# LiuTaowen-Tony/xKV

Measured on NVIDIA B200. Metric: KV GB/s compressed (prefill, xKV-4, Llama-3.1-8B 64K), higher is better.
Workload: dtype bf16

## Files before the change

include/xkv_b200.h:

```cpp
#ifndef XKV_B200_H_
#define XKV_B200_H_

#include <stddef.h>
#include <stdint.h>

#ifdef __cplusplus
extern "C" {
#endif

#if defined(__GNUC__)
#define XKV_API __attribute__((visibility("default")))
#else
#define XKV_API
#endif

#define XKV_MAX_GROUP_LAYERS 16
#define XKV_MAX_GEMM_PROBLEMS 16
#define XKV_MAX_BATCH 16
#define XKV_MAX_LAYER_MAPS 64

XKV_API const char* xkv_last_error(void);
XKV_API int xkv_version(void);
XKV_API int64_t xkv_launch_count(void);

// ... 5 lines not shown
                     void* stream);

typedef struct xkv_gemm_problem {
  int32_t M, N, K;
  int32_t num_terms;
  int32_t a_mn_major;
  int32_t b_mn_major;
  const void* A[3];
  const void* B[3];
  int64_t lda, ldb;
  uint8_t term_a[6], term_b[6];
  void* D;
  int64_t ldd;
  int32_t out_bf16;
  int32_t out_transposed;
  int32_t sym_upper;
  int32_t split_k;
  int64_t split_stride;
  int32_t accum_phases;
  const int32_t* run_if;
  int32_t a_layers, b_layers, layer_cols;
  const void* A_layer[XKV_MAX_GROUP_LAYERS];
  const void* B_layer[XKV_MAX_GROUP_LAYERS];
} xkv_gemm_problem;
XKV_API int xkv_gemm_grouped(const xkv_gemm_problem* problems_host, int num_problems, void* stream);
XKV_API size_t xkv_gemm_problem_size(void);
XKV_API void xkv_gemm_set_gram_pair(int on);

XKV_API int xkv_reduce_slabs(const float* slabs, int num_slabs, int64_t slab_stride, int rows, int cols, int64_t ld,
                     int symmetrize, float* out, int64_t ld_out, void* stream);
XKV_API int xkv_reduce_slabs_batched(const float* const* slabs_host, float* const* out_host, int batch, int num_slabs,
                                     int64_t slab_stride, int rows, int cols, int64_t ld, int symmetrize,
                                     int64_t ld_out, void* stream);
XKV_API int xkv_split_bf16(const float* x, int rows, int cols, int64_t ld, void* hi, void* mid, void* lo,
                   int64_t ld_out, void* stream);
XKV_API int xkv_split_bf16_batched(const float* const* x_host, void* const* hi_host, void* const* mid_host,
                                   void* const* lo_host, int batch, int rows, int cols, int64_t ld, int64_t ld_out,
                                   void* stream);
XKV_API int xkv_symmetrize_split_bf16(const float* const* slabs_host, int batch, int num_slabs, int64_t slab_stride,
                                      int n, int64_t ld, void* const* hi_host, void* const* mid_host,
                                      void* const* lo_host, int64_t ld_out, void* stream);
XKV_API size_t xkv_gram_packed_elems(int n);
XKV_API int xkv_gram_pack_upper(const float* full, int n, int64_t ld, float* packed, void* stream);
XKV_API int xkv_gram_unpack_upper(const float* packed, int n, float* full, int64_t ld, void* stream);
XKV_API int xkv_fill_gaussian_bf16(void* out, int rows, int cols, int64_t ld, uint64_t seed, void* stream);
XKV_API int xkv_normalize_rows(float* const* Y_host, void* const* hi_host, void* const* mid_host,
                               void* const* lo_host, int batch, int rows, int cols, int64_t ld, int64_t ld_out,
                               void* stream);
XKV_API int xkv_shift_normalize_rows(float* const* Y_host, const float* const* Q_host, float* shift_dev,
                                     float* const* rdiag_host, int rdiag_first, void* const* hi_host,
// ... 120 lines not shown
```

xkv_b200/_lib.py:

```python
from __future__ import annotations

import ctypes as C
import os
from typing import Optional

_LIB_PATH = os.environ.get("XKV_B200_LIB") or os.path.join(os.path.dirname(os.path.abspath(__file__)), "libxkv_b200.so")
_lib: Optional[C.CDLL] = None

MAX_GROUP_LAYERS = 16
MAX_GEMM_PROBLEMS = 16
MAX_BATCH = 16


class XkvError(RuntimeError):
    """Raised when a C-ABI call returns a non-zero status (mirrors the reference's Python exceptions)."""


class GemmProblem(C.Structure):

    _fields_ = [
        ("M", C.c_int32),
        ("N", C.c_int32),
        ("K", C.c_int32),
        ("num_terms", C.c_int32),
        ("a_mn_major", C.c_int32),
        ("b_mn_major", C.c_int32),
        ("A", C.c_void_p * 3),
        ("B", C.c_void_p * 3),
        ("lda", C.c_int64),
        ("ldb", C.c_int64),
        ("term_a", C.c_uint8 * 6),
        ("term_b", C.c_uint8 * 6),
        ("D", C.c_void_p),
        ("ldd", C.c_int64),
        ("out_bf16", C.c_int32),
        ("out_transposed", C.c_int32),
        ("sym_upper", C.c_int32),
        ("split_k", C.c_int32),
        ("split_stride", C.c_int64),
        ("accum_phases", C.c_int32),
        ("run_if", C.c_void_p),
        ("a_layers", C.c_int32),
        ("b_layers", C.c_int32),
        ("layer_cols", C.c_int32),
        ("A_layer", C.c_void_p * MAX_GROUP_LAYERS),
        ("B_layer", C.c_void_p * MAX_GROUP_LAYERS),
    ]


class AppendProblem(C.Structure):

    _fields_ = [("x_new", C.c_void_p), ("V", C.c_void_p), ("a_out", C.c_void_p), ("ldx", C.c_int64), ("ldv", C.c_int64),
                ("lda", C.c_int64), ("n", C.c_int32), ("r", C.c_int32)]


class FactorizeOptions(C.Structure):

    _fields_ = [
        ("power_iters", C.c_int32),
        ("oversample", C.c_int32),
        ("first_passes", C.c_int32),
        ("passes", C.c_int32),
        ("final_passes", C.c_int32),
        ("window", C.c_int32),
        ("jacobi_sweeps", C.c_int32),
        ("rayleigh_ritz", C.c_int32),
        ("want_sigma", C.c_int32),
        ("gram_split_k", C.c_int32),
        ("gram_chunk_tokens", C.c_int32),
# ... 45 lines not shown
    "xkv_convert_bf16": (_i, [_vp, _i, _i, _i64, _vp, _i64, _vp, _i64, _vp]),
    "xkv_sqrt_clamp": (_i, [_vp, _vp, _i, _vp]),
    "xkv_factorize_default_options": (None, [C.POINTER(FactorizeOptions)]),
    "xkv_factorize_workspace_bytes": (_sz, [_i, _i, _i, _i, C.POINTER(FactorizeOptions)]),
    "xkv_factorize_sigma_count": (_i, [_i, C.POINTER(FactorizeOptions)]),
    "xkv_decode_workspace_bytes": (_sz, [_i, _i, _i, _i]),
    "xkv_decode_attention": (_i, [_vp, _i, _i, _i, _vp, _i64, _i, _vp, _i64, _vp, _i64, _i, _vp, _i64, _i, _vp, _vp, _i64,
                                  _vp, _vp, _i, _i64, _i64, _f, _vp, _vp, _sz, _vp]),
    "xkv_decode_attention_lse": (_i, [_vp, _i, _i, _i, _vp, _i64, _i, _vp, _i64, _vp, _i64, _i, _vp, _i64, _i, _vp, _vp,
                                      _i64, _vp, _vp, _i, _i64, _i64, _f, _vp, _vp, _sz, _vp, _vp]),
    "xkv_decode_absorbed_workspace_bytes": (_sz, [_i, _i, _i]),
    "xkv_decode_absorbed": (_i, [_vp, _i, _vp, _i64, _i, _i, _vp, _vp, _vp, _i64, _i, _f, _vp, _vp, _vp, _sz, _vp]),
    "xkv_decode_force_tiled": (None, [_i]),
    "xkv_decode_set_variant": (None, [_i]),
    "xkv_decode_set_stages": (None, [_i]),
    "xkv_rope_bf16": (_i, [_vp, _i64, _i, _i, _i, _vp, _vp, _i64, _vp]),
    "xkv_append_workspace_bytes": (_sz, [_i, _i, _i]),
    "xkv_append_project": (_i, [_vp, _i64, _i, _vp, _i64, _i, _i, _vp, _i64, _vp, _sz, _vp]),
    "xkv_append_project_batch": (_i, [C.POINTER(AppendProblem), _i, _i, _vp, _sz, _vp]),
    "xkv_slerp_workspace_bytes": (_sz, [_i64]),
    "xkv_slerp_merge": (_i, [_vp, _vp, _i64, _i, _i64, _f, _f, _vp, _vp, _i64, _vp, _sz, _vp]),
    "xkv_gemm_problem_size": (C.c_size_t, []),
    "xkv_gemm_set_gram_pair": (None, [_i]),
    "xkv_factorize_groups": (_i, [_pp, _i, _i, _i, _i, _i64, _i, C.POINTER(FactorizeOptions), _pp, _pp, _pp, _pp, _vp, _sz,
                                  _pp, _vp]),
    "xkv_factorize_workspace_bytes_mixed": (_sz, [_i, _i, _i, _vp, C.POINTER(FactorizeOptions)]),
    "xkv_factorize_groups_mixed": (_i, [_pp, _i, _i, _i, _i, _i64, _vp, C.POINTER(FactorizeOptions), _pp, _pp, _pp, _pp, _vp,
                                        _sz, _pp, _vp]),
    "xkv_factorize_batch_mixed": (_i, [_pp, _i, _i, _i, _i64, _vp, C.POINTER(FactorizeOptions), _pp, _pp, _pp, _pp, _vp, _sz,
                                       _pp, _vp]),
    "xkv_factorize_batch": (_i, [_pp, _i, _i, _i, _i64, _i, C.POINTER(FactorizeOptions), _pp, _pp, _pp, _pp, _pp, _i,
                                 _vp, _sz, _pp, _vp]),
}


def lib_path() -> str:
    return _LIB_PATH


def load() -> C.CDLL:
    global _lib
    if _lib is not None:
        return _lib
    if not os.path.exists(_LIB_PATH):
        raise XkvError(
            f"{_LIB_PATH} not found: build it with `python -c 'import __graft_entry__ as g; g.build()'` "
# ... 16 lines not shown
```

xkv_b200/csrc/xkv_factorize.cu:

```cuda
#include <cuda_bf16.h>

#include <vector>

#include "xkv_host.h"

namespace xkv {

static inline size_t align_up(size_t x, size_t a) { return (x + a - 1) / a * a; }
static inline int round_up_int(int x, int k) { return (x + k - 1) / k * k; }

struct Bump {
  char* base;
  size_t off, cap;
  bool overflow;
  void* take(size_t bytes) {
    off = align_up(off, 1024);
    void* p = base ? base + off : nullptr;
    off += bytes;
    if (base && off > cap) overflow = true;
    return p;
  }
  float* f32(size_t n) { return static_cast<float*>(take(n * 4)); }
  void* bf16(size_t n) { return take(n * 2); }
};
// ... 411 lines not shown
                                               o.pivot_floor, stream));
          }
          if (o.heavy_redo && pp > 0 && shift < o.shifts[0]) {
            BatchRowsScope rows(l_rows);
            XKV_TRY(xkv_pass_flags(P.linv, B, lmax, lmax, 2.f * shift, P.redo_flags, stream));
            xkv_set_launch_predicate(P.redo_flags);
            int rc2 = xkv_reduce_slabs_batched(P.s_slabs, P.s_mat, B, P.sk, static_cast<long long>(lmax) * lmax, lmax, lmax, lmax,
                                               1, lmax, stream);
            if (!rc2)
              rc2 = xkv_cholesky_inverse_limbs(P.s_mat, P.linv, h0, h1, nt > 3 ? h2 : nullptr, B, lmax, lmax, lmax, o.shifts[0],
                                               o.pivot_floor, stream);
            xkv_set_launch_predicate(cond ? P.pass_flags : nullptr);
            if (rc2) return rc2;
          }
        }
        if (track) {
          BatchRowsScope rows(l_rows);
          XKV_TRY(xkv_rdiag_update(P.rdiag, P.linv, B, lmax, lmax, stream));
        }
        for (int b = 0; b < B; ++b) {
          xkv_gemm_problem p = swap_roles(problem(P.linv_l[b][0], P.linv_l[b][1], P.linv_l[b][2], lmax, 0, P.lh[b], P.lm[b],
                                                  P.ll[b], nn, 1, cond ? cur[b] : nxt[b], nn, l[b], n, l[b],
                                                  (o.solve_terms == 3 && !final_call) ? 3 : nt));
          p.run_if = cond ? P.pass_flags + b : nullptr;
          ps.push_back(p);
        }
        XKV_TRY(run_gemms(ps, stream));
        return 0;
      }();
      if (cond) xkv_set_launch_predicate(nullptr);
      if (rc) return rc;
      if (!cond) swap_bufs();
    }
    return 0;
  };
  auto apply_gram = [&](int nterms) -> int {
    for (int b = 0; b < B; ++b)
      ps.push_back(swap_roles(problem(P.lh[b], P.lm[b], P.ll[b], nn, 0, P.g_limb[b][0], P.g_limb[b][1], P.g_limb[b][2], nn, 0,
                                      nxt[b], nn, l[b], n, n, nterms)));
    XKV_TRY(run_gemms(ps, stream));
    swap_bufs();
    return 0;
  };

  for (int b = 0; b < B; ++b) XKV_TRY(xkv_fill_gaussian_bf16(P.lh[b], l[b], n, nn, o.seed + 7919ull * b, stream));
  XKV_TRY(apply_gram(1));
// ... 175 lines not shown
```

xkv_b200/csrc/xkv_gemm.cu:

```cuda
#include <cstdlib>

#include "xkv_common.cuh"
#include "xkv_host.h"

namespace xkv {

constexpr int BM = 128;
constexpr int BN = 256;
constexpr int BK = 64;
constexpr int STAGES = 4;
constexpr int A_TILE_BYTES = BM * BK * 2;
constexpr int B_TILE_BYTES = BN * BK * 2;
constexpr int STAGE_BYTES = A_TILE_BYTES + B_TILE_BYTES;
constexpr int CHUNK_BYTES = 64 * BK * 2;
constexpr int GEMM_THREADS = 192;
constexpr int TMEM_COLS = 256;
constexpr size_t GEMM_SMEM_BYTES = STAGES * STAGE_BYTES + 1024  + 256 ;

struct alignas(64) GemmProb {
  CUtensorMap a_map[3];
  CUtensorMap b_map[3];
  void* D;
  long long ldd;
  long long split_stride;
  int M, N, K;
  int nterms;
  int tiles_m, tiles_n, ntiles;
  int split_k, kblocks_per_split, nkb;
  int cta_begin;
  int bn;
  int na, nb;
  unsigned char la[3], lb[3];
  unsigned char sa[3], sb[3];
  int pstages;
  int out_bf16, out_transposed, sym_upper;
  unsigned char ta[6], tb[6];
  const int* run_if;
  int phases;
  int a_layers, a_layer_begin, b_layers, b_layer_begin, layer_cols;
};
struct GemmParams {
  int nprob;
  int pair_stages;
  GemmProb p[XKV_MAX_GEMM_PROBLEMS];
  CUtensorMap layer_maps[XKV_MAX_LAYER_MAPS];
};

__device__ __forceinline__ const CUtensorMap* layer_map(const GemmParams& P, int begin, int layers, int layer_cols, int col,
                                                        int& col_in_layer) {
  int li = col / layer_cols;
  li = li < layers ? li : layers - 1;
  col_in_layer = col - li * layer_cols;
  return &P.layer_maps[begin + li];
}

template <int A_MN, int B_MN>
__global__ void __launch_bounds__(GEMM_THREADS, 1) gemm_kernel(const __grid_constant__ GemmParams P) {
  extern __shared__ uint8_t smem_raw[];
  uint8_t* smem = reinterpret_cast<uint8_t*>((reinterpret_cast<uintptr_t>(smem_raw) + 1023) & ~uintptr_t(1023));
  uint64_t* full_bar = reinterpret_cast<uint64_t*>(smem + STAGES * STAGE_BYTES);
  uint64_t* empty_bar = full_bar + STAGES;
  uint64_t* tmem_full_bar = empty_bar + STAGES;
  uint64_t* tmem_empty_bar = tmem_full_bar + 2;
  uint32_t* tmem_slot = reinterpret_cast<uint32_t*>(tmem_empty_bar + 2);

  const int warp = threadIdx.x >> 5;
  const int lane = threadIdx.x & 31;

  int pi = 0;
  while (pi + 1 < P.nprob && static_cast<int>(blockIdx.x) >= P.p[pi + 1].cta_begin) ++pi;
  const GemmProb& pr = P.p[pi];
  if (pr.run_if != nullptr && *pr.run_if == 0) return;
  const int local = static_cast<int>(blockIdx.x) - pr.cta_begin;
  const int split = local / pr.ntiles;
  int t = local - split * pr.ntiles;
  int tm, tn;
  if (pr.sym_upper) {
    tm = 0;
    tn = 0;
    for (int i = 0; i < pr.tiles_m; ++i) {
      const int first = (i * BM) / BN;
      const int cnt = pr.tiles_n - first;
      if (t < cnt) {
        tm = i;
        tn = first + t;
        break;
      }
      t -= cnt;
    }
  } else {
    tm = t / pr.tiles_n;
    tn = t - tm * pr.tiles_n;
  }
  const int m0 = tm * BM;
  const int n0 = tn * BN;
  const int kb0 = split * pr.kblocks_per_split;
  const int kb1 = min(kb0 + pr.kblocks_per_split, pr.nkb);
  const int nk = max(kb1 - kb0, 0);
  const int niter = nk * pr.nterms;
  const int nph = max(1, min(pr.phases, nk));
  const uint32_t tmem_cols = nph > 1 ? 2 * TMEM_COLS : TMEM_COLS;

  if (warp == 0 && lane == 0) {
    for (int i = 0; i < STAGES; ++i) {
      mbar_init(&full_bar[i], 1);
      mbar_init(&empty_bar[i], 1);
    }
    mbar_init(&tmem_full_bar[0], 1);
    mbar_init(&tmem_full_bar[1], 1);
    mbar_init(&tmem_empty_bar[0], 4);
    mbar_init(&tmem_empty_bar[1], 4);
    mbar_fence_init();
    for (int i = 0; i < 3; ++i) {
      tma_prefetch_desc(&pr.a_map[i]);
      tma_prefetch_desc(&pr.b_map[i]);
    }
  }
  if (warp == 1) tmem_alloc(tmem_slot, tmem_cols);
  tc_fence_before();
  __syncthreads();
  tc_fence_after();
  const uint32_t tmem_base = *tmem_slot;

  if (warp == 0) {
    const CUtensorMap* a_chunk_map[BM / 64];
    int a_chunk_col[BM / 64];
    const CUtensorMap* b_chunk_map[BN / 64];
    int b_chunk_col[BN / 64];
#pragma unroll
    for (int c = 0; c < BM / 64; ++c) {
      a_chunk_col[c] = m0 + 64 * c;
      a_chunk_map[c] = (A_MN && pr.a_layers) ? layer_map(P, pr.a_layer_begin, pr.a_layers, pr.layer_cols, m0 + 64 * c, a_chunk_col[c]) : nullptr;
    }
#pragma unroll
    for (int c = 0; c < BN / 64; ++c) {
      b_chunk_col[c] = n0 + 64 * c;
      b_chunk_map[c] = (B_MN && pr.b_layers) ? layer_map(P, pr.b_layer_begin, pr.b_layers, pr.layer_cols, n0 + 64 * c, b_chunk_col[c]) : nullptr;
    }
    int ka_layer = 0, ka_col = 0, kb_layer = 0, kb_col = 0;
    if (!A_MN && pr.a_layers) {
      ka_layer = (kb0 * BK) / pr.layer_cols;
      ka_col = kb0 * BK - ka_layer * pr.layer_cols;
    }
    if (!B_MN && pr.b_layers) {
      kb_layer = (kb0 * BK) / pr.layer_cols;
      kb_col = kb0 * BK - kb_layer * pr.layer_cols;
    }
    if (elect_one()) {
      int s = 0, term = 0, kb = kb0;
      uint32_t ph = 0;
      for (int it = 0; it < niter; ++it) {
        const CUtensorMap* amap = &pr.a_map[pr.ta[term]];
        const CUtensorMap* bmap = &pr.b_map[pr.tb[term]];
        uint8_t* sA = smem + s * STAGE_BYTES;
        uint8_t* sB = sA + A_TILE_BYTES;
        mbar_wait(&empty_bar[s], ph ^ 1u);
        mbar_expect_tx(&full_bar[s], STAGE_BYTES);
        if (A_MN == 0) {
          if (pr.a_layers)
            tma_load_2d(sA, &P.layer_maps[pr.a_layer_begin + min(ka_layer, pr.a_layers - 1)], &full_bar[s],
                        ka_layer < pr.a_layers ? ka_col : pr.layer_cols, m0);
          else
            tma_load_2d(sA, amap, &full_bar[s], kb * BK, m0);
        } else {
#pragma unroll
          for (int c = 0; c < BM / 64; ++c)
            tma_load_2d(sA + c * CHUNK_BYTES, a_chunk_map[c] ? a_chunk_map[c] : amap, &full_bar[s], a_chunk_col[c], kb * BK);
        }
        if (B_MN == 0) {
          if (pr.b_layers)
            tma_load_2d(sB, &P.layer_maps[pr.b_layer_begin + min(kb_layer, pr.b_layers - 1)], &full_bar[s],
                        kb_layer < pr.b_layers ? kb_col : pr.layer_cols, n0);
          else
            tma_load_2d(sB, bmap, &full_bar[s], kb * BK, n0);
        } else {
#pragma unroll
          for (int c = 0; c < BN / 64; ++c)
            tma_load_2d(sB + c * CHUNK_BYTES, b_chunk_map[c] ? b_chunk_map[c] : bmap, &full_bar[s], b_chunk_col[c], kb * BK);
        }
        if (!A_MN && pr.a_layers && (ka_col += BK) >= pr.layer_cols) {
          ka_col -= pr.layer_cols;
          ++ka_layer;
        }
        if (!B_MN && pr.b_layers && (kb_col += BK) >= pr.layer_cols) {
          kb_col -= pr.layer_cols;
          ++kb_layer;
        }
        if (++term == pr.nterms) {
          term = 0;
          ++kb;
        }
        if (++s == STAGES) {
          s = 0;
          ph ^= 1u;
        }
      }
    }
    __syncwarp();
  } else if (warp == 1) {
    constexpr uint32_t idesc = umma_idesc_bf16(BM, BN, A_MN, B_MN);
    constexpr uint64_t kStageStep = STAGE_BYTES >> 4;
    constexpr uint64_t kAStep = (A_MN ? 2048 : 32) >> 4, kBStep = (B_MN ? 2048 : 32) >> 4;
    if (elect_one()) {
      const uint32_t a_base0 = smem_u32(smem);
      const uint64_t a_desc0 = A_MN ? umma_desc_sw128(a_base0, CHUNK_BYTES, 1024) : umma_desc_sw128(a_base0, 16, 1024);
      const uint64_t b_desc0 = B_MN ? umma_desc_sw128(a_base0 + A_TILE_BYTES, CHUNK_BYTES, 1024)
                                    : umma_desc_sw128(a_base0 + A_TILE_BYTES, 16, 1024);
      uint64_t a_desc = a_desc0, b_desc = b_desc0;
      int s = 0;
      uint32_t ph = 0;
      int it = 0;
      for (int phs = 0; phs < nph; ++phs) {
        const uint32_t acc = tmem_base + static_cast<uint32_t>(phs & 1) * TMEM_COLS;
        if (phs >= 2) {
          mbar_wait(&tmem_empty_bar[phs & 1], static_cast<uint32_t>(((phs >> 1) - 1) & 1));
          tc_fence_after();
        }
        const int it_end = (nph == 1) ? niter : static_cast<int>((static_cast<long long>(nk) * (phs + 1)) / nph) * pr.nterms;
        const int it_begin = it;
        for (; it < it_end; ++it) {
          mbar_wait(&full_bar[s], ph);
          tc_fence_after();
          umma_bf16_ss(acc, a_desc, b_desc, idesc, it > it_begin ? 1u : 0u);
          umma_bf16_ss(acc, a_desc + kAStep, b_desc + kBStep, idesc, 1u);
          umma_bf16_ss(acc, a_desc + 2 * kAStep, b_desc + 2 * kBStep, idesc, 1u);
          umma_bf16_ss(acc, a_desc + 3 * kAStep, b_desc + 3 * kBStep, idesc, 1u);
          umma_commit(&empty_bar[s]);
          a_desc += kStageStep;
          b_desc += kStageStep;
          if (++s == STAGES) {
            s = 0;
            ph ^= 1u;
            a_desc = a_desc0;
            b_desc = b_desc0;
          }
        }
        umma_commit(&tmem_full_bar[phs & 1]);
      }
    }
    __syncwarp();
  } else {
    const int q = warp & 3;
    const int row = m0 + q * 32 + lane;
    const bool row_ok = row < pr.M;
    float* outf = reinterpret_cast<float*>(pr.D) + static_cast<long long>(split) * pr.split_stride;
    __nv_bfloat16* outh = reinterpret_cast<__nv_bfloat16*>(pr.D) + static_cast<long long>(split) * pr.split_stride;
    const bool vec_ok = (pr.ldd % 8 == 0) && ((reinterpret_cast<uintptr_t>(pr.D) & 15) == 0) &&
                        ((pr.split_stride % 8) == 0);
#pragma unroll 1
    for (int phs = 0; phs < nph; ++phs) {
    float4 pre[8];
    auto prefetch = [&](int c) -> bool {
      const int col0 = n0 + c * 32;
      if (!(phs > 0 && row_ok && vec_ok && c < BN / 32 && col0 + 32 <= pr.N)) return false;
      const float4* src = reinterpret_cast<const float4*>(outf + static_cast<long long>(row) * pr.ldd + col0);
#pragma unroll
      for (int j = 0; j < 8; ++j) pre[j] = src[j];
      return true;
    };
    bool have_pre = prefetch(0);
    mbar_wait(&tmem_full_bar[phs & 1], static_cast<uint32_t>((phs >> 1) & 1));
    tc_fence_after();
    const uint32_t acc = tmem_base + static_cast<uint32_t>(phs & 1) * TMEM_COLS;
#pragma unroll 1
    for (int c = 0; c < BN / 32; ++c) {
      const int col0 = n0 + c * 32;
      if (col0 >= pr.N) break;
      uint32_t v[32];
      __syncwarp();
      if (niter > 0) {
        tmem_ld_32x32(acc + (static_cast<uint32_t>(q * 32) << 16) + static_cast<uint32_t>(c * 32), v);
        float4 cur[8];
        const bool have_cur = have_pre;
#pragma unroll
        for (int j = 0; j < 8; ++j) cur[j] = pre[j];
        have_pre = prefetch(c + 1);
        tmem_ld_wait();
        if (have_cur) {
#pragma unroll
          for (int j = 0; j < 8; ++j) {
            v[4 * j] = __float_as_uint(__uint_as_float(v[4 * j]) + cur[j].x);
            v[4 * j + 1] = __float_as_uint(__uint_as_float(v[4 * j + 1]) + cur[j].y);
            v[4 * j + 2] = __float_as_uint(__uint_as_float(v[4 * j + 2]) + cur[j].z);
            v[4 * j + 3] = __float_as_uint(__uint_as_float(v[4 * j + 3]) + cur[j].w);
          }
        } else if (phs > 0 && row_ok) {
          const float* src = outf + static_cast<long long>(row) * pr.ldd + col0;
#pragma unroll
// ... 100 lines not shown
  const int local = (static_cast<int>(blockIdx.x) - pr.cta_begin) >> 1;
  const int split = local / pr.ntiles;
  int t = local - split * pr.ntiles;
  int tm = 0, tn = 0;
  if (pr.sym_upper) {
    for (int i = 0; i < pr.tiles_m; ++i) {
      const int cnt = pr.tiles_n - i;
      if (t < cnt) {
        tm = i;
        tn = i + t;
        break;
      }
      t -= cnt;
    }
  } else {
    tm = t / pr.tiles_n;
    tn = t - tm * pr.tiles_n;
  }
  const int m0 = tm * PG_BM + crank * BM;
  const int n0 = tn * bn;
  const int nb0 = n0 + crank * (bn >> 1);
  const int n_end = min(pr.N, n0 + bn);
  const int kb0 = split * pr.kblocks_per_split;
  const int kb1 = min(kb0 + pr.kblocks_per_split, pr.nkb);
  const int nk = max(kb1 - kb0, 0);
  const int niter = nk * pr.nterms;
  const int nph = max(1, min(pr.phases, nk));
  const uint32_t tmem_cols = nph > 1 ? 2 * TMEM_COLS : TMEM_COLS;
  const uint32_t b_bytes = B_MN ? static_cast<uint32_t>(PG_B_BYTES) : static_cast<uint32_t>(bn >> 1) * (BK * 2);

  if (warp == 0 && lane == 0) {
    for (int i = 0; i < nstages; ++i) {
      mbar_init(&full_bar[i], 1);
      mbar_init(&empty_bar[i], 1);
    }
    mbar_init(&tmem_full_bar[0], 1);
    mbar_init(&tmem_full_bar[1], 1);
    mbar_init(&tmem_empty_bar[0], 8);
    mbar_init(&tmem_empty_bar[1], 8);
    mbar_fence_init();
    tma_prefetch_desc(&pr.a_map[pr.ta[0]]);
    tma_prefetch_desc(&pr.b_map[pr.tb[0]]);
  }
  if (warp == 1) tmem_alloc_pair(tmem_slot, tmem_cols);
  tc_fence_before();
  __syncthreads();
  cluster_sync_all();
// ... 225 lines not shown
              if (row_ok && col0 + j < n_end)
                outh[static_cast<long long>(col0 + j) * pr.ldd + row] = __float2bfloat16_rn(__uint_as_float(v[j]));
          }
        }
      }
      if (phs + 2 < nph) {
        tc_fence_before();
        __syncwarp();
        if (lane == 0) mbar_arrive_cluster(tempty0 + static_cast<uint32_t>((phs & 1) * 8));
      }
    }
  }

  tc_fence_before();
  __syncthreads();
  cluster_sync_all();
  if (warp == 1) {
    tc_fence_after();
    tmem_dealloc_pair(tmem_base, tmem_cols);
  }
}

static int g_gram_pair = 1;

static int pair_bn(const xkv_gemm_problem& p) {
  if (!g_gram_pair) return 0;
  const int rem = p.M % PG_BM;
  if (!(p.M >= 2048 || rem == 0 || rem > BM)) return 0;
  if (p.sym_upper) return (p.a_mn_major && p.b_mn_major && p.M == p.N) ? BN : 0;
  if (p.b_mn_major) return BN;
  const int ntn = (p.N + BN - 1) / BN;
  const int w = (p.N + ntn - 1) / ntn;
  return (w + 15) & ~15;
}

static int build_problem(const xkv_gemm_problem& in, GemmProb& out, int& cta_cursor, GemmParams& params, int& map_cursor,
                         int pair_n = 0) {
  const bool pair = pair_n > 0;
  const int bn = pair ? pair_n : BN;
  XKV_REQUIRE(in.M > 0 && in.N > 0 && in.K > 0, "gemm: empty problem M=%d N=%d K=%d", in.M, in.N, in.K);
  XKV_REQUIRE(in.num_terms >= 1 && in.num_terms <= 6, "gemm: num_terms=%d out of range", in.num_terms);
  XKV_REQUIRE(in.lda % 8 == 0 && in.ldb % 8 == 0, "gemm: lda/ldb must be multiples of 8 elements");
  XKV_REQUIRE(in.split_k >= 1, "gemm: split_k must be >= 1");
  XKV_REQUIRE(in.D != nullptr, "gemm: null output");
  std::memset(&out, 0, sizeof(out));
  bool used_a[3] = {false, false, false}, used_b[3] = {false, false, false};
  for (int t = 0; t < in.num_terms; ++t) {
    XKV_REQUIRE(in.term_a[t] < 3 && in.term_b[t] < 3, "gemm: limb index out of range");
    used_a[in.term_a[t]] = true;
    used_b[in.term_b[t]] = true;
    out.ta[t] = in.term_a[t];
    out.tb[t] = in.term_b[t];
  }
  XKV_REQUIRE(in.a_layers >= 0 && in.a_layers <= XKV_MAX_GROUP_LAYERS && in.b_layers >= 0 && in.b_layers <= XKV_MAX_GROUP_LAYERS,
              "gemm: at most %d layers per operand", XKV_MAX_GROUP_LAYERS);
  if (in.a_layers > 0 || in.b_layers > 0) {
    XKV_REQUIRE(in.num_terms == 1, "gemm: layered operands take one term");
    XKV_REQUIRE(in.layer_cols > 0 && in.layer_cols % 64 == 0, "gemm: layer_cols=%d must be a positive multiple of 64", in.layer_cols);
  }
  for (int side = 0; side < 2; ++side) {
    const int layers = side == 0 ? in.a_layers : in.b_layers;
    if (layers == 0) continue;
    const void* const* ptrs = side == 0 ? in.A_layer : in.B_layer;
    const bool mn = side == 0 ? in.a_mn_major != 0 : in.b_mn_major != 0;
    const long long ld = side == 0 ? in.lda : in.ldb;
    const int other = side == 0 ? in.M : in.N;
    if (side == 1 && in.a_layers == in.b_layers && in.a_mn_major && in.b_mn_major && in.lda == in.ldb &&
        std::memcmp(in.A_layer, in.B_layer, sizeof(void*) * layers) == 0) {
      out.b_layer_begin = out.a_layer_begin;
      continue;
    }
    (side == 0 ? out.a_layer_begin : out.b_layer_begin) = map_cursor;
    for (int i = 0; i < layers; ++i) {
      XKV_REQUIRE(ptrs[i] != nullptr && (reinterpret_cast<uintptr_t>(ptrs[i]) & 15) == 0, "gemm: layer %d null or unaligned", i);
      XKV_REQUIRE(map_cursor < XKV_MAX_LAYER_MAPS, "gemm: more than %d layer matrices in one launch", XKV_MAX_LAYER_MAPS);
      int rc;
      if (!mn)
        rc = encode_tmap_2d_bf16(&params.layer_maps[map_cursor++], ptrs[i], in.layer_cols, other, ld, BK,
                                 side == 0 ? BM : (pair ? bn / 2 : BN));
      else
        rc = encode_tmap_2d_bf16(&params.layer_maps[map_cursor++], ptrs[i], in.layer_cols, in.K, ld, 64, BK);
      if (rc) return rc;
    }
  }
  out.a_layers = in.a_layers;
  out.b_layers = in.b_layers;
  out.layer_cols = in.layer_cols;
  XKV_REQUIRE(in.a_layers == 0 || (in.a_mn_major ? in.M : in.K) <= in.a_layers * in.layer_cols, "gemm: layered A narrower than the problem");
  XKV_REQUIRE(in.b_layers == 0 || (in.b_mn_major ? in.N : in.K) <= in.b_layers * in.layer_cols, "gemm: layered B narrower than the problem");
  for (int i = 0; i < 3; ++i) {
    const void* a = in.a_layers > 0 ? in.A_layer[0] : (used_a[i] ? in.A[i] : in.A[in.term_a[0]]);
    const void* b = in.b_layers > 0 ? in.B_layer[0] : (used_b[i] ? in.B[i] : in.B[in.term_b[0]]);
    XKV_REQUIRE(a != nullptr && b != nullptr, "gemm: null operand limb %d", i);
    XKV_REQUIRE((reinterpret_cast<uintptr_t>(a) & 15) == 0 && (reinterpret_cast<uintptr_t>(b) & 15) == 0,
                "gemm: operands must be 16-byte aligned");
    int rc = 0;
    if (in.a_layers > 0)
      out.a_map[i] = params.layer_maps[out.a_layer_begin];
    else if (!in.a_mn_major)
      rc = encode_tmap_2d_bf16(&out.a_map[i], a, in.K, in.M, in.lda, BK, BM);
    else
      rc = encode_tmap_2d_bf16(&out.a_map[i], a, in.M, in.K, in.lda, 64, BK);
    if (rc) return rc;
    if (in.b_layers > 0)
      out.b_map[i] = params.layer_maps[out.b_layer_begin];
    else if (!in.b_mn_major)
      rc = encode_tmap_2d_bf16(&out.b_map[i], b, in.K, in.N, in.ldb, BK, pair ? bn / 2 : BN);
    else
      rc = encode_tmap_2d_bf16(&out.b_map[i], b, in.N, in.K, in.ldb, 64, BK);
    if (rc) return rc;
  }
  out.D = in.D;
  out.ldd = in.ldd;
  out.split_stride = in.split_stride;
  out.M = in.M;
  out.N = in.N;
  out.K = in.K;
  out.nterms = in.num_terms;
  const int bm = pair ? PG_BM : BM;
  out.bn = bn;
  out.tiles_m = (in.M + bm - 1) / bm;
  out.tiles_n = (in.N + bn - 1) / bn;
  out.sym_upper = in.sym_upper ? 1 : 0;
  if (out.sym_upper) {
    int cnt = 0;
    for (int i = 0; i < out.tiles_m; ++i) cnt += out.tiles_n - (i * bm) / bn;
    out.ntiles = cnt;
  } else {
    out.ntiles = out.tiles_m * out.tiles_n;
  }
  for (int i = 0; i < 3; ++i) {
    if (used_a[i]) {
      out.sa[i] = static_cast<unsigned char>(out.na);
      out.la[out.na++] = static_cast<unsigned char>(i);
    }
    if (used_b[i]) {
      out.sb[i] = static_cast<unsigned char>(out.nb);
      out.lb[out.nb++] = static_cast<unsigned char>(i);
    }
  }
  out.nkb = (in.K + BK - 1) / BK;
  out.split_k = in.split_k;
  out.kblocks_per_split = (out.nkb + in.split_k - 1) / in.split_k;
  out.out_bf16 = in.out_bf16 ? 1 : 0;
  out.out_transposed = in.out_transposed ? 1 : 0;
  out.run_if = in.run_if;
  out.phases = in.accum_phases > 1 ? in.accum_phases : 1;
  XKV_REQUIRE(out.phases == 1 || (!in.out_bf16 && !in.out_transposed),
              "gemm: accum_phases > 1 needs a plain fp32 output");
  out.cta_begin = cta_cursor;
  cta_cursor += out.ntiles * out.split_k * (pair ? 2 : 1);
  return 0;
}

bool& gemm_low_priority() {
  static thread_local bool low = false;
  return low;
}

template <int A_MN, int B_MN>
static int launch_pair_variant(GemmParams& params, int grid, cudaStream_t stream) {
  auto kern = gemm_pair_kernel<A_MN, B_MN>;
  static PerDevice<bool> configured;
  if (!configured()) {
    XKV_CHECK_CUDA(cudaFuncSetAttribute(kern, cudaFuncAttributeMaxDynamicSharedMemorySize,
                                        static_cast<int>(pg_smem_bytes(PG_MAX_STAGES))));
    configured() = true;
  }
  params.pair_stages = (g_gram_pair >= 3 && g_gram_pair <= PG_MAX_STAGES) ? g_gram_pair : PG_STAGES;
  for (int i = 0; i < params.nprob; ++i) {
    const int stage = (params.p[i].na + params.p[i].nb) * PG_A_BYTES;
    const int st = params.pair_stages * PG_STAGE_BYTES / stage;
// ... 3 lines not shown
  std::memset(&cfg, 0, sizeof(cfg));
  cfg.gridDim = dim3(grid, 1, 1);
  cfg.blockDim = dim3(GEMM_THREADS, 1, 1);
  cfg.dynamicSmemBytes = pg_smem_bytes(params.pair_stages);
  cfg.stream = stream;
  cudaLaunchAttribute attr[2];
  attr[0].id = cudaLaunchAttributeClusterDimension;
  attr[0].val.clusterDim.x = 2;
  attr[0].val.clusterDim.y = 1;
  attr[0].val.clusterDim.z = 1;
  cfg.numAttrs = 1;
  if (gemm_low_priority()) {
    attr[1].id = cudaLaunchAttributePriority;
    attr[1].val.priority = 0;
    cfg.numAttrs = 2;
  }
  cfg.attrs = attr;
  XKV_CHECK_CUDA(cudaLaunchKernelEx(&cfg, kern, params));
  XKV_LAUNCHED();
  return 0;
}

template <int A_MN, int B_MN>
static int launch_variant(const GemmParams& params, int grid, cudaStream_t stream) {
  auto kern = gemm_kernel<A_MN, B_MN>;
  static PerDevice<bool> configured;
  if (!configured()) {
    XKV_CHECK_CUDA(cudaFuncSetAttribute(kern, cudaFuncAttributeMaxDynamicSharedMemorySize,
                                        static_cast<int>(GEMM_SMEM_BYTES)));
    configured() = true;
  }
  if (gemm_low_priority()) {
    cudaLaunchConfig_t cfg;
    std::memset(&cfg, 0, sizeof(cfg));
    cfg.gridDim = dim3(grid, 1, 1);
    cfg.blockDim = dim3(GEMM_THREADS, 1, 1);
    cfg.dynamicSmemBytes = GEMM_SMEM_BYTES;
    cfg.stream = stream;
    cudaLaunchAttribute attr[1];
    attr[0].id = cudaLaunchAttributePriority;
    attr[0].val.priority = 0;
    cfg.attrs = attr;
    cfg.numAttrs = 1;
    XKV_CHECK_CUDA(cudaLaunchKernelEx(&cfg, kern, params));
  } else {
    kern<<<grid, GEMM_THREADS, GEMM_SMEM_BYTES, stream>>>(params);
  }
  XKV_LAUNCHED();
  return 0;
}

}

extern "C" size_t xkv_gemm_problem_size(void) { return sizeof(xkv_gemm_problem); }
extern "C" void xkv_gemm_set_gram_pair(int on) { xkv::g_gram_pair = on < 0 ? 0 : on; }

extern "C" int xkv_gemm_grouped(const xkv_gemm_problem* problems, int num_problems, void* stream) {
  using namespace xkv;
  XKV_REQUIRE(problems != nullptr && num_problems >= 1, "gemm: no problems");
  XKV_REQUIRE(num_problems <= XKV_MAX_GEMM_PROBLEMS, "gemm: at most %d problems per launch", XKV_MAX_GEMM_PROBLEMS);
  const int a_mn = problems[0].a_mn_major ? 1 : 0;
  const int b_mn = problems[0].b_mn_major ? 1 : 0;
  static thread_local GemmParams params;
  params.nprob = num_problems;
  int cursor = 0, map_cursor = 0;
  bool pair = true;
  for (int i = 0; i < num_problems; ++i) pair = pair && pair_bn(problems[i]) > 0;
  for (int i = 0; i < num_problems; ++i) {
    XKV_REQUIRE((problems[i].a_mn_major ? 1 : 0) == a_mn && (problems[i].b_mn_major ? 1 : 0) == b_mn,
                "gemm: all problems of one launch must share operand majors");
    int rc = build_problem(problems[i], params.p[i], cursor, params, map_cursor, pair ? pair_bn(problems[i]) : 0);
    if (rc) return rc;
  }
  cudaStream_t st = as_stream(stream);
  if (pair) {
    if (!a_mn && !b_mn) return launch_pair_variant<0, 0>(params, cursor, st);
    if (!a_mn && b_mn) return launch_pair_variant<0, 1>(params, cursor, st);
    if (a_mn && !b_mn) return launch_pair_variant<1, 0>(params, cursor, st);
// ... 8 lines not shown
```

xkv_b200/ops.py:

```python
from __future__ import annotations

import ctypes as C
from typing import List, Optional, Sequence, Tuple

import torch

from . import _lib
from ._lib import GemmProblem, check

TERMS_1 = ((0, 0),)
TERMS_3 = ((0, 0), (0, 1), (1, 0))
TERMS_6 = ((0, 0), (0, 1), (1, 0), (1, 1), (0, 2), (2, 0))


def _stream() -> C.c_void_p:
    return C.c_void_p(torch.cuda.current_stream().cuda_stream)


def _require_cuda(*tensors: torch.Tensor) -> None:
    cur = None
    for t in tensors:
        if t is None:
            continue
        if not t.is_cuda:
# ... 37 lines not shown
    sb, sh, ss, sd = layers[0].stride()
    ptrs = (C.c_void_p * g)(*[t.data_ptr() for t in layers])
    check(lib.xkv_unpack_group(C.c_void_p(x.data_ptr()), g, bs, h, s, d, sb, sh, ss, ptrs, _stream()))


def make_problem(
    a_limbs: Sequence[torch.Tensor],
    b_limbs: Sequence[torch.Tensor],
    out: torch.Tensor,
    *,
    M: int,
    N: int,
    K: int,
    a_mn_major: bool = False,
    b_mn_major: bool = False,
    terms: Sequence[Tuple[int, int]] = TERMS_1,
    out_transposed: bool = False,
    sym_upper: bool = False,
    split_k: int = 1,
    split_stride: int = 0,
    accum_phases: int = 1,
    a_layers: Optional[Sequence[torch.Tensor]] = None,
    b_layers: Optional[Sequence[torch.Tensor]] = None,
) -> GemmProblem:
    p = GemmProblem()
    p.M, p.N, p.K = M, N, K
    p.num_terms = len(terms)
    p.a_mn_major, p.b_mn_major = int(a_mn_major), int(b_mn_major)
    for i in range(3):
        a = a_limbs[i] if i < len(a_limbs) else None
        b = b_limbs[i] if i < len(b_limbs) else None
        p.A[i] = a.data_ptr() if a is not None else None
        p.B[i] = b.data_ptr() if b is not None else None
    for t in list(a_limbs) + list(b_limbs) + list(a_layers or []) + list(b_layers or []):
        if t is not None and (t.dtype != torch.bfloat16 or t.stride(-1) != 1):
            raise _lib.XkvError("gemm operands must be bf16 with unit inner stride")
    for side, layers in (("a", a_layers), ("b", b_layers)):
        if not layers:
            continue
        if len(layers) > _lib.MAX_GROUP_LAYERS or any(t.shape != layers[0].shape or t.stride() != layers[0].stride() for t in layers):
            raise _lib.XkvError("gemm: layered operands must be equally shaped and strided (at most 16 layers)")
        setattr(p, side + "_layers", len(layers))
        p.layer_cols = layers[0].shape[1]
        arr = p.A_layer if side == "a" else p.B_layer
        for i, t in enumerate(layers):
            arr[i] = t.data_ptr()
    p.lda = (a_layers[0] if a_layers else a_limbs[0]).stride(0)
    p.ldb = (b_layers[0] if b_layers else b_limbs[0]).stride(0)
    for t, (ta, tb) in enumerate(terms):
        p.term_a[t], p.term_b[t] = ta, tb
    if out.dtype not in (torch.float32, torch.bfloat16) or out.stride(-1) != 1:
        raise _lib.XkvError("gemm output must be fp32 or bf16 with unit inner stride")
    p.D = out.data_ptr()
    p.ldd = out.stride(-2)
    p.out_bf16 = int(out.dtype == torch.bfloat16)
    p.out_transposed = int(out_transposed)
    p.sym_upper = int(sym_upper)
    p.split_k = split_k
    p.split_stride = split_stride
    p.accum_phases = accum_phases
    return p


def gemm_grouped(problems: Sequence[GemmProblem]) -> None:
    lib = _lib.load()
    arr = (GemmProblem * len(problems))(*problems)
    check(lib.xkv_gemm_grouped(arr, len(problems), _stream()))


def _ptr(t: Optional[torch.Tensor]) -> C.c_void_p:
    return C.c_void_p(t.data_ptr() if t is not None else None)


def _ptr_array(ts: Optional[Sequence[Optional[torch.Tensor]]]):
    if ts is None:
        return None
    return (C.c_void_p * len(ts))(*[(t.data_ptr() if t is not None else None) for t in ts])


def reduce_slabs(slabs: torch.Tensor, out: torch.Tensor, symmetrize: bool = False) -> None:
    _require_cuda(slabs, out)
    s, rows, cols = slabs.shape
    check(_lib.load().xkv_reduce_slabs(_ptr(slabs), s, slabs.stride(0), rows, cols, slabs.stride(1), int(symmetrize),
# ... 270 lines not shown
```

Measured before the change: 238.3.

## Load limbs once per stage, shrink tiles for symmetric grams, skip zero K-blocks

Reworks the GEMM producer/consumer pipeline so that each stage loads every distinct A/B limb once and issues all multi-term products from those shared tiles, where the old code reloaded tiles for each term. The stage count now follows the ring size. Symmetric Gram products use a 128-wide N tile so diagonal tiles can reuse the A tile as B, and a new b_lower flag truncates the K loop for lower-triangular B operands in the Cholesky-QR solve. A runtime knob selects the mode. This adds complexity, variable stage counts and more tiles for the narrow-N cases.

```diff
diff --git a/include/xkv_b200.h b/include/xkv_b200.h
--- a/include/xkv_b200.h
+++ b/include/xkv_b200.h
@@ -51,10 +51,12 @@
   int32_t a_layers, b_layers, layer_cols;
   const void* A_layer[XKV_MAX_GROUP_LAYERS];
   const void* B_layer[XKV_MAX_GROUP_LAYERS];
+  int32_t b_lower;
 } xkv_gemm_problem;
 XKV_API int xkv_gemm_grouped(const xkv_gemm_problem* problems_host, int num_problems, void* stream);
 XKV_API size_t xkv_gemm_problem_size(void);
 XKV_API void xkv_gemm_set_gram_pair(int on);
+XKV_API void xkv_gemm_set_cholqr_tiles(int mode);
 
 XKV_API int xkv_reduce_slabs(const float* slabs, int num_slabs, int64_t slab_stride, int rows, int cols, int64_t ld,
                      int symmetrize, float* out, int64_t ld_out, void* stream);
diff --git a/xkv_b200/_lib.py b/xkv_b200/_lib.py
--- a/xkv_b200/_lib.py
+++ b/xkv_b200/_lib.py
@@ -45,6 +45,7 @@
         ("layer_cols", C.c_int32),
         ("A_layer", C.c_void_p * MAX_GROUP_LAYERS),
         ("B_layer", C.c_void_p * MAX_GROUP_LAYERS),
+        ("b_lower", C.c_int32),
     ]
 
 
@@ -136,6 +137,7 @@
     "xkv_slerp_merge": (_i, [_vp, _vp, _i64, _i, _i64, _f, _f, _vp, _vp, _i64, _vp, _sz, _vp]),
     "xkv_gemm_problem_size": (C.c_size_t, []),
     "xkv_gemm_set_gram_pair": (None, [_i]),
+    "xkv_gemm_set_cholqr_tiles": (None, [_i]),
     "xkv_factorize_groups": (_i, [_pp, _i, _i, _i, _i, _i64, _i, C.POINTER(FactorizeOptions), _pp, _pp, _pp, _pp, _vp, _sz,
                                   _pp, _vp]),
     "xkv_factorize_workspace_bytes_mixed": (_sz, [_i, _i, _i, _vp, C.POINTER(FactorizeOptions)]),
diff --git a/xkv_b200/csrc/xkv_factorize.cu b/xkv_b200/csrc/xkv_factorize.cu
--- a/xkv_b200/csrc/xkv_factorize.cu
+++ b/xkv_b200/csrc/xkv_factorize.cu
@@ -457,6 +457,7 @@
           xkv_gemm_problem p = swap_roles(problem(P.linv_l[b][0], P.linv_l[b][1], P.linv_l[b][2], lmax, 0, P.lh[b], P.lm[b],
                                                   P.ll[b], nn, 1, cond ? cur[b] : nxt[b], nn, l[b], n, l[b],
                                                   (o.solve_terms == 3 && !final_call) ? 3 : nt));
+          p.b_lower = 1;
           p.run_if = cond ? P.pass_flags + b : nullptr;
           ps.push_back(p);
         }
diff --git a/xkv_b200/csrc/xkv_gemm.cu b/xkv_b200/csrc/xkv_gemm.cu
--- a/xkv_b200/csrc/xkv_gemm.cu
+++ b/xkv_b200/csrc/xkv_gemm.cu
@@ -8,14 +8,14 @@
 constexpr int BM = 128;
 constexpr int BN = 256;
 constexpr int BK = 64;
-constexpr int STAGES = 4;
 constexpr int A_TILE_BYTES = BM * BK * 2;
 constexpr int B_TILE_BYTES = BN * BK * 2;
-constexpr int STAGE_BYTES = A_TILE_BYTES + B_TILE_BYTES;
+constexpr int RING_BYTES = 4 * (A_TILE_BYTES + B_TILE_BYTES);
+constexpr int MAX_STAGES = 6;
 constexpr int CHUNK_BYTES = 64 * BK * 2;
 constexpr int GEMM_THREADS = 192;
 constexpr int TMEM_COLS = 256;
-constexpr size_t GEMM_SMEM_BYTES = STAGES * STAGE_BYTES + 1024  + 256 ;
+constexpr size_t GEMM_SMEM_BYTES = RING_BYTES + 1024  + 256 ;
 
 struct alignas(64) GemmProb {
   CUtensorMap a_map[3];
@@ -33,6 +33,9 @@
   unsigned char la[3], lb[3];
   unsigned char sa[3], sb[3];
   int pstages;
+  int per_term;
+  int diag_shared;
+  int b_lower;
   int out_bf16, out_transposed, sym_upper;
   unsigned char ta[6], tb[6];
   const int* run_if;
@@ -58,9 +61,9 @@
 __global__ void __launch_bounds__(GEMM_THREADS, 1) gemm_kernel(const __grid_constant__ GemmParams P) {
   extern __shared__ uint8_t smem_raw[];
   uint8_t* smem = reinterpret_cast<uint8_t*>((reinterpret_cast<uintptr_t>(smem_raw) + 1023) & ~uintptr_t(1023));
-  uint64_t* full_bar = reinterpret_cast<uint64_t*>(smem + STAGES * STAGE_BYTES);
-  uint64_t* empty_bar = full_bar + STAGES;
-  uint64_t* tmem_full_bar = empty_bar + STAGES;
+  uint64_t* full_bar = reinterpret_cast<uint64_t*>(smem + RING_BYTES);
+  uint64_t* empty_bar = full_bar + MAX_STAGES;
+  uint64_t* tmem_full_bar = empty_bar + MAX_STAGES;
   uint64_t* tmem_empty_bar = tmem_full_bar + 2;
   uint32_t* tmem_slot = reinterpret_cast<uint32_t*>(tmem_empty_bar + 2);
 
@@ -71,6 +74,14 @@
   while (pi + 1 < P.nprob && static_cast<int>(blockIdx.x) >= P.p[pi + 1].cta_begin) ++pi;
   const GemmProb& pr = P.p[pi];
   if (pr.run_if != nullptr && *pr.run_if == 0) return;
+  const int bn = pr.bn;
+  const int nstages = pr.pstages;
+  const bool per_term = pr.per_term != 0;
+  const int nsa = per_term ? 1 : pr.na;
+  const int nsb = per_term ? 1 : pr.nb;
+  const uint32_t b_slot_bytes = static_cast<uint32_t>(bn) * (BK * 2);
+  const uint32_t stage_bytes = static_cast<uint32_t>(nsa) * A_TILE_BYTES + static_cast<uint32_t>(nsb) * b_slot_bytes;
+  const int sps = per_term ? pr.nterms : 1;
   const int local = static_cast<int>(blockIdx.x) - pr.cta_begin;
   const int split = local / pr.ntiles;
   int t = local - split * pr.ntiles;
@@ -79,7 +90,7 @@
     tm = 0;
     tn = 0;
     for (int i = 0; i < pr.tiles_m; ++i) {
-      const int first = (i * BM) / BN;
+      const int first = (i * BM) / bn;
       const int cnt = pr.tiles_n - first;
       if (t < cnt) {
         tm = i;
@@ -93,16 +104,18 @@
     tn = t - tm * pr.tiles_n;
   }
   const int m0 = tm * BM;
-  const int n0 = tn * BN;
+  const int n0 = tn * bn;
+  const bool diag = !A_MN && !B_MN && pr.diag_shared && m0 == n0;
   const int kb0 = split * pr.kblocks_per_split;
-  const int kb1 = min(kb0 + pr.kblocks_per_split, pr.nkb);
+  const int nkb = pr.b_lower ? min(pr.nkb, (min(pr.N, n0 + bn) + BK - 1) / BK) : pr.nkb;
+  const int kb1 = min(kb0 + pr.kblocks_per_split, nkb);
   const int nk = max(kb1 - kb0, 0);
-  const int niter = nk * pr.nterms;
+  const int niter = nk * sps;
   const int nph = max(1, min(pr.phases, nk));
   const uint32_t tmem_cols = nph > 1 ? 2 * TMEM_COLS : TMEM_COLS;
 
   if (warp == 0 && lane == 0) {
-    for (int i = 0; i < STAGES; ++i) {
+    for (int i = 0; i < nstages; ++i) {
       mbar_init(&full_bar[i], 1);
       mbar_init(&empty_bar[i], 1);
     }
@@ -127,6 +140,7 @@
     int a_chunk_col[BM / 64];
     const CUtensorMap* b_chunk_map[BN / 64];
     int b_chunk_col[BN / 64];
+    const int nbc = bn / 64;
 #pragma unroll
     for (int c = 0; c < BM / 64; ++c) {
       a_chunk_col[c] = m0 + 64 * c;
@@ -135,7 +149,7 @@
 #pragma unroll
     for (int c = 0; c < BN / 64; ++c) {
       b_chunk_col[c] = n0 + 64 * c;
-      b_chunk_map[c] = (B_MN && pr.b_layers) ? layer_map(P, pr.b_layer_begin, pr.b_layers, pr.layer_cols, n0 + 64 * c, b_chunk_col[c]) : nullptr;
+      b_chunk_map[c] = (B_MN && pr.b_layers && c < nbc) ? layer_map(P, pr.b_layer_begin, pr.b_layers, pr.layer_cols, n0 + 64 * c, b_chunk_col[c]) : nullptr;
     }
     int ka_layer = 0, ka_col = 0, kb_layer = 0, kb_col = 0;
     if (!A_MN && pr.a_layers) {
@@ -149,34 +163,42 @@
     if (elect_one()) {
       int s = 0, term = 0, kb = kb0;
       uint32_t ph = 0;
+      const uint32_t tx = diag ? static_cast<uint32_t>(nsa) * A_TILE_BYTES : stage_bytes;
       for (int it = 0; it < niter; ++it) {
-        const CUtensorMap* amap = &pr.a_map[pr.ta[term]];
-        const CUtensorMap* bmap = &pr.b_map[pr.tb[term]];
-        uint8_t* sA = smem + s * STAGE_BYTES;
-        uint8_t* sB = sA + A_TILE_BYTES;
+        uint8_t* sA = smem + s * stage_bytes;
+        uint8_t* sB = sA + nsa * A_TILE_BYTES;
         mbar_wait(&empty_bar[s], ph ^ 1u);
-        mbar_expect_tx(&full_bar[s], STAGE_BYTES);
-        if (A_MN == 0) {
-          if (pr.a_layers)
-            tma_load_2d(sA, &P.layer_maps[pr.a_layer_begin + min(ka_layer, pr.a_layers - 1)], &full_bar[s],
-                        ka_layer < pr.a_layers ? ka_col : pr.layer_cols, m0);
-          else
-            tma_load_2d(sA, amap, &full_bar[s], kb * BK, m0);
-        } else {
-#pragma unroll
-          for (int c = 0; c < BM / 64; ++c)
-            tma_load_2d(sA + c * CHUNK_BYTES, a_chunk_map[c] ? a_chunk_map[c] : amap, &full_bar[s], a_chunk_col[c], kb * BK);
-        }
-        if (B_MN == 0) {
-          if (pr.b_layers)
-            tma_load_2d(sB, &P.layer_maps[pr.b_layer_begin + min(kb_layer, pr.b_layers - 1)], &full_bar[s],
-                        kb_layer < pr.b_layers ? kb_col : pr.layer_cols, n0);
-          else
-            tma_load_2d(sB, bmap, &full_bar[s], kb * BK, n0);
-        } else {
-#pragma unroll
-          for (int c = 0; c < BN / 64; ++c)
-            tma_load_2d(sB + c * CHUNK_BYTES, b_chunk_map[c] ? b_chunk_map[c] : bmap, &full_bar[s], b_chunk_col[c], kb * BK);
+        mbar_expect_tx(&full_bar[s], tx);
+        for (int i = 0; i < nsa; ++i) {
+          const CUtensorMap* amap = &pr.a_map[per_term ? pr.ta[term] : pr.la[i]];
+          uint8_t* dst = sA + i * A_TILE_BYTES;
+          if (A_MN == 0) {
+            if (pr.a_layers)
+              tma_load_2d(dst, &P.layer_maps[pr.a_layer_begin + min(ka_layer, pr.a_layers - 1)], &full_bar[s],
+                          ka_layer < pr.a_layers ? ka_col : pr.layer_cols, m0);
+            else
+              tma_load_2d(dst, amap, &full_bar[s], kb * BK, m0);
+          } else {
+#pragma unroll
+            for (int c = 0; c < BM / 64; ++c)
+              tma_load_2d(dst + c * CHUNK_BYTES, a_chunk_map[c] ? a_chunk_map[c] : amap, &full_bar[s], a_chunk_col[c], kb * BK);
+          }
+        }
+        for (int i = 0; i < (diag ? 0 : nsb); ++i) {
+          const CUtensorMap* bmap = &pr.b_map[per_term ? pr.tb[term] : pr.lb[i]];
+          uint8_t* dst = sB + i * b_slot_bytes;
+          if (B_MN == 0) {
+            if (pr.b_layers)
+              tma_load_2d(dst, &P.layer_maps[pr.b_layer_begin + min(kb_layer, pr.b_layers - 1)], &full_bar[s],
+                          kb_layer < pr.b_layers ? kb_col : pr.layer_cols, n0);
+            else
+              tma_load_2d(dst, bmap, &full_bar[s], kb * BK, n0);
+          } else {
+#pragma unroll
+            for (int c = 0; c < BN / 64; ++c)
+              if (c < nbc)
+                tma_load_2d(dst + c * CHUNK_BYTES, b_chunk_map[c] ? b_chunk_map[c] : bmap, &full_bar[s], b_chunk_col[c], kb * BK);
+          }
         }
         if (!A_MN && pr.a_layers && (ka_col += BK) >= pr.layer_cols) {
           ka_col -= pr.layer_cols;
@@ -186,11 +208,11 @@
           kb_col -= pr.layer_cols;
           ++kb_layer;
         }
-        if (++term == pr.nterms) {
+        if (++term == sps) {
           term = 0;
           ++kb;
         }
-        if (++s == STAGES) {
+        if (++s == nstages) {
           s = 0;
           ph ^= 1u;
         }
@@ -198,16 +220,21 @@
     }
     __syncwarp();
   } else if (warp == 1) {
-    constexpr uint32_t idesc = umma_idesc_bf16(BM, BN, A_MN, B_MN);
-    constexpr uint64_t kStageStep = STAGE_BYTES >> 4;
+    const uint32_t idesc = umma_idesc_bf16(BM, 0, A_MN, B_MN) | (static_cast<uint32_t>(bn >> 3) << 17);
     constexpr uint64_t kAStep = (A_MN ? 2048 : 32) >> 4, kBStep = (B_MN ? 2048 : 32) >> 4;
+    constexpr uint64_t kASlot = A_TILE_BYTES >> 4;
     if (elect_one()) {
+      const uint64_t kStageStep = stage_bytes >> 4;
+      const uint64_t kBSlot = b_slot_bytes >> 4;
       const uint32_t a_base0 = smem_u32(smem);
       const uint64_t a_desc0 = A_MN ? umma_desc_sw128(a_base0, CHUNK_BYTES, 1024) : umma_desc_sw128(a_base0, 16, 1024);
-      const uint64_t b_desc0 = B_MN ? umma_desc_sw128(a_base0 + A_TILE_BYTES, CHUNK_BYTES, 1024)
-                                    : umma_desc_sw128(a_base0 + A_TILE_BYTES, 16, 1024);
+      const uint64_t b_desc0 = diag ? a_desc0
+                               : B_MN ? umma_desc_sw128(a_base0 + nsa * A_TILE_BYTES, CHUNK_BYTES, 1024)
+                                      : umma_desc_sw128(a_base0 + nsa * A_TILE_BYTES, 16, 1024);
+      const uint64_t kBSlotUsed = diag ? kASlot : kBSlot;
+      const unsigned char* bslot = diag ? pr.sa : pr.sb;
       uint64_t a_desc = a_desc0, b_desc = b_desc0;
-      int s = 0;
+      int s = 0, term = 0;
       uint32_t ph = 0;
       int it = 0;
       for (int phs = 0; phs < nph; ++phs) {
@@ -216,19 +243,25 @@
           mbar_wait(&tmem_empty_bar[phs & 1], static_cast<uint32_t>(((phs >> 1) - 1) & 1));
           tc_fence_after();
         }
-        const int it_end = (nph == 1) ? niter : static_cast<int>((static_cast<long long>(nk) * (phs + 1)) / nph) * pr.nterms;
+        const int it_end = (nph == 1) ? niter : static_cast<int>((static_cast<long long>(nk) * (phs + 1)) / nph) * sps;
         const int it_begin = it;
         for (; it < it_end; ++it) {
           mbar_wait(&full_bar[s], ph);
           tc_fence_after();
-          umma_bf16_ss(acc, a_desc, b_desc, idesc, it > it_begin ? 1u : 0u);
-          umma_bf16_ss(acc, a_desc + kAStep, b_desc + kBStep, idesc, 1u);
-          umma_bf16_ss(acc, a_desc + 2 * kAStep, b_desc + 2 * kBStep, idesc, 1u);
-          umma_bf16_ss(acc, a_desc + 3 * kAStep, b_desc + 3 * kBStep, idesc, 1u);
+          const int t0 = per_term ? term : 0, t1 = per_term ? term + 1 : pr.nterms;
+          for (int t = t0; t < t1; ++t) {
+            const uint64_t ad = per_term ? a_desc : a_desc + kASlot * pr.sa[pr.ta[t]];
+            const uint64_t bd = per_term ? b_desc : b_desc + kBSlotUsed * bslot[pr.tb[t]];
+            umma_bf16_ss(acc, ad, bd, idesc, (it > it_begin || t > t0) ? 1u : 0u);
+            umma_bf16_ss(acc, ad + kAStep, bd + kBStep, idesc, 1u);
+            umma_bf16_ss(acc, ad + 2 * kAStep, bd + 2 * kBStep, idesc, 1u);
+            umma_bf16_ss(acc, ad + 3 * kAStep, bd + 3 * kBStep, idesc, 1u);
+          }
           umma_commit(&empty_bar[s]);
+          if (++term == sps) term = 0;
           a_desc += kStageStep;
           b_desc += kStageStep;
-          if (++s == STAGES) {
+          if (++s == nstages) {
             s = 0;
             ph ^= 1u;
             a_desc = a_desc0;
@@ -252,7 +285,7 @@
     float4 pre[8];
     auto prefetch = [&](int c) -> bool {
       const int col0 = n0 + c * 32;
-      if (!(phs > 0 && row_ok && vec_ok && c < BN / 32 && col0 + 32 <= pr.N)) return false;
+      if (!(phs > 0 && row_ok && vec_ok && c < bn / 32 && col0 + 32 <= pr.N)) return false;
       const float4* src = reinterpret_cast<const float4*>(outf + static_cast<long long>(row) * pr.ldd + col0);
 #pragma unroll
       for (int j = 0; j < 8; ++j) pre[j] = src[j];
@@ -263,7 +296,7 @@
     tc_fence_after();
     const uint32_t acc = tmem_base + static_cast<uint32_t>(phs & 1) * TMEM_COLS;
 #pragma unroll 1
-    for (int c = 0; c < BN / 32; ++c) {
+    for (int c = 0; c < bn / 32; ++c) {
       const int col0 = n0 + c * 32;
       if (col0 >= pr.N) break;
       uint32_t v[32];
@@ -410,7 +443,8 @@
   const int nb0 = n0 + crank * (bn >> 1);
   const int n_end = min(pr.N, n0 + bn);
   const int kb0 = split * pr.kblocks_per_split;
-  const int kb1 = min(kb0 + pr.kblocks_per_split, pr.nkb);
+  const int nkb = pr.b_lower ? min(pr.nkb, (n_end + BK - 1) / BK) : pr.nkb;
+  const int kb1 = min(kb0 + pr.kblocks_per_split, nkb);
   const int nk = max(kb1 - kb0, 0);
   const int niter = nk * pr.nterms;
   const int nph = max(1, min(pr.phases, nk));
@@ -682,6 +716,11 @@
 }
 
 static int g_gram_pair = 1;
+static int g_cholqr_tiles = 1;
+
+static int single_bn(const xkv_gemm_problem& p) {
+  return (g_cholqr_tiles && p.sym_upper && !p.a_mn_major && !p.b_mn_major) ? BM : BN;
+}
 
 static int pair_bn(const xkv_gemm_problem& p) {
   if (!g_gram_pair) return 0;
@@ -697,7 +736,7 @@
 static int build_problem(const xkv_gemm_problem& in, GemmProb& out, int& cta_cursor, GemmParams& params, int& map_cursor,
                          int pair_n = 0) {
   const bool pair = pair_n > 0;
-  const int bn = pair ? pair_n : BN;
+  const int bn = pair ? pair_n : single_bn(in);
   XKV_REQUIRE(in.M > 0 && in.N > 0 && in.K > 0, "gemm: empty problem M=%d N=%d K=%d", in.M, in.N, in.K);
   XKV_REQUIRE(in.num_terms >= 1 && in.num_terms <= 6, "gemm: num_terms=%d out of range", in.num_terms);
   XKV_REQUIRE(in.lda % 8 == 0 && in.ldb % 8 == 0, "gemm: lda/ldb must be multiples of 8 elements");
@@ -737,7 +776,7 @@
       int rc;
       if (!mn)
         rc = encode_tmap_2d_bf16(&params.layer_maps[map_cursor++], ptrs[i], in.layer_cols, other, ld, BK,
-                                 side == 0 ? BM : (pair ? bn / 2 : BN));
+                                 side == 0 ? BM : (pair ? bn / 2 : bn));
       else
         rc = encode_tmap_2d_bf16(&params.layer_maps[map_cursor++], ptrs[i], in.layer_cols, in.K, ld, 64, BK);
       if (rc) return rc;
@@ -765,7 +804,7 @@
     if (in.b_layers > 0)
       out.b_map[i] = params.layer_maps[out.b_layer_begin];
     else if (!in.b_mn_major)
-      rc = encode_tmap_2d_bf16(&out.b_map[i], b, in.K, in.N, in.ldb, BK, pair ? bn / 2 : BN);
+      rc = encode_tmap_2d_bf16(&out.b_map[i], b, in.K, in.N, in.ldb, BK, pair ? bn / 2 : bn);
     else
       rc = encode_tmap_2d_bf16(&out.b_map[i], b, in.N, in.K, in.ldb, 64, BK);
     if (rc) return rc;
@@ -808,6 +847,14 @@
   out.phases = in.accum_phases > 1 ? in.accum_phases : 1;
   XKV_REQUIRE(out.phases == 1 || (!in.out_bf16 && !in.out_transposed),
               "gemm: accum_phases > 1 needs a plain fp32 output");
+  XKV_REQUIRE(!in.b_lower || (!in.b_mn_major && in.b_layers == 0 && in.split_k == 1 && out.phases == 1),
+              "gemm: b_lower needs a K-major B without layers, split_k = 1 and accum_phases <= 1");
+  out.b_lower = (in.b_lower && g_cholqr_tiles) ? 1 : 0;
+  bool same = !pair && bn == BM && in.sym_upper && !in.a_mn_major && !in.b_mn_major && in.a_layers == 0 &&
+              in.b_layers == 0 && in.M == in.N && in.lda == in.ldb;
+  for (int i = 0; i < 3 && same; ++i)
+    if (used_b[i]) same = used_a[i] && in.A[i] == in.B[i];
+  out.diag_shared = same ? 1 : 0;
   out.cta_begin = cta_cursor;
   cta_cursor += out.ntiles * out.split_k * (pair ? 2 : 1);
   return 0;
@@ -857,13 +904,22 @@
 }
 
 template <int A_MN, int B_MN>
-static int launch_variant(const GemmParams& params, int grid, cudaStream_t stream) {
+static int launch_variant(GemmParams& params, int grid, cudaStream_t stream) {
   auto kern = gemm_kernel<A_MN, B_MN>;
   static PerDevice<bool> configured;
   if (!configured()) {
     XKV_CHECK_CUDA(cudaFuncSetAttribute(kern, cudaFuncAttributeMaxDynamicSharedMemorySize,
                                         static_cast<int>(GEMM_SMEM_BYTES)));
     configured() = true;
+  }
+  for (int i = 0; i < params.nprob; ++i) {
+    GemmProb& pr = params.p[i];
+    const int b_slot = pr.bn * BK * 2;
+    const int distinct = pr.na * A_TILE_BYTES + pr.nb * b_slot;
+    pr.per_term = (g_cholqr_tiles != 1 || RING_BYTES / distinct < 2) ? 1 : 0;
+    if (pr.per_term) pr.diag_shared = 0;
+    const int st = RING_BYTES / (pr.per_term ? A_TILE_BYTES + b_slot : distinct);
+    pr.pstages = st > MAX_STAGES ? MAX_STAGES : st;
   }
   if (gemm_low_priority()) {
     cudaLaunchConfig_t cfg;
@@ -889,6 +945,7 @@
 
 extern "C" size_t xkv_gemm_problem_size(void) { return sizeof(xkv_gemm_problem); }
 extern "C" void xkv_gemm_set_gram_pair(int on) { xkv::g_gram_pair = on < 0 ? 0 : on; }
+extern "C" void xkv_gemm_set_cholqr_tiles(int mode) { xkv::g_cholqr_tiles = (mode >= 0 && mode <= 2) ? mode : 1; }
 
 extern "C" int xkv_gemm_grouped(const xkv_gemm_problem* problems, int num_problems, void* stream) {
   using namespace xkv;
diff --git a/xkv_b200/ops.py b/xkv_b200/ops.py
--- a/xkv_b200/ops.py
+++ b/xkv_b200/ops.py
@@ -83,6 +83,7 @@
     accum_phases: int = 1,
     a_layers: Optional[Sequence[torch.Tensor]] = None,
     b_layers: Optional[Sequence[torch.Tensor]] = None,
+    b_lower: bool = False,
 ) -> GemmProblem:
     p = GemmProblem()
     p.M, p.N, p.K = M, N, K
@@ -120,6 +121,7 @@
     p.split_k = split_k
     p.split_stride = split_stride
     p.accum_phases = accum_phases
+    p.b_lower = int(b_lower)
     return p
 
 
```

Result: faster. 242.6 (median of 6 runs) (+1.8%).
